# whwh747/A-Low-Texture-Robust-Hybrid-Feature-Based-Visual-Odometry

Measured on AMD Instinct MI355X. Metric: RGB-D frames/sec (640×480, 1k ORB + LSD + PEAC) at 1/2/4/8 GPUs, higher is better.
Workload: dtype u8/u16 integer + f32/f64; 1 GPU; 640x480 synthetic RGB-D, 1000 ORB (quota; 3/4 std + 1/4 lowtex scenes) + LSD lines + PEAC planes, 8192 frames per GPU per step (std640); frames_per_gpu=8192, parallelism=frames sharded, 1 rank(s), no data-path collective, distinct_frames=256, resident_bytes_per_frame_estimate=21100000

## Files before the change

a-low-texture-robust-hybrid-feature-based-visual-odometry_amd/__init__.py:

```python
import ctypes as C
import os
import subprocess
import numpy as np

_HERE = os.path.dirname(os.path.abspath(__file__))
_CSRC = os.path.join(_HERE, "csrc")
_LIBPATH = os.environ.get("HVO_LIB") or os.path.join(_CSRC, "libhvo.so")
_LIB = None
_LOADED_BEFORE_TORCH = False

HVO_OK = 0
STAGE_ORB, STAGE_LSD, STAGE_PLANES, STAGE_ALL = 1, 2, 4, 7
SLAB_LABELS = 1
STAGE_LSD_CULL = 8
STAGE_LINES3D, STAGE_VP, STAGE_PLANE_TAIL, STAGE_GRIDS = 16, 32, 64, 128
STAGE_FRAME = 1 | 2 | 8 | 4 | 16 | 32 | 64 | 128
LINE_MATCH_NNR, LINE_MATCH_BF, LINE_MATCH_DOUBLE = 0, 1, 2

KEYPOINT_DT = np.dtype([("x", "<f4"), ("y", "<f4"), ("size", "<f4"), ("angle", "<f4"),
                        ("response", "<f4"), ("octave", "<i4"), ("class_id", "<i4")])
KEYLINE_DT = np.dtype([("angle", "<f4"), ("class_id", "<i4"), ("octave", "<i4"),
                       ("pt_x", "<f4"), ("pt_y", "<f4"), ("response", "<f4"), ("size", "<f4"),
                       ("sx", "<f4"), ("sy", "<f4"), ("ex", "<f4"), ("ey", "<f4"),
                       ("sox", "<f4"), ("soy", "<f4"), ("eox", "<f4"), ("eoy", "<f4"),
# ... 1004 lines not shown

    def normals_lpvo(self, depth):
        depth = np.ascontiguousarray(depth, np.uint16); h, w = depth.shape
        cap = ((h + 14) // 15) * ((w + 14) // 15)
        nrm = np.zeros((cap, 3)); dz = np.zeros(cap, np.float32); px = np.zeros((cap, 2), np.int32); n = C.c_int(0)
        self._chk(lib().hvo_normals_lpvo(self.h, _p(depth), w, h, depth.strides[0], _p(nrm), _p(dz), _p(px), cap, C.byref(n)), "normals_lpvo")
        return nrm[: n.value], dz[: n.value], px[: n.value]

    def surface_normals(self, depth):
        depth = np.ascontiguousarray(depth, np.uint16); h, w = depth.shape
        cap = (((h + 2) // 3) // 2) * (((w + 2) // 3) // 2)
        out = np.zeros(max(cap, 1), SURFACE_NORMAL_DT); n = C.c_int(0)
        self._chk(lib().hvo_surface_normals(self.h, _p(depth), w, h, depth.strides[0], _p(out), cap, C.byref(n)), "surface_normals")
        return out[: n.value].copy()

    def peac_stats(self, frame=0):
        L = lib()
        L.hvo_debug_peac_stats.argtypes = [C.c_void_p, C.c_int, C.c_void_p]; L.hvo_debug_peac_stats.restype = C.c_int
        m = np.zeros(16, np.int32)
        self._chk(L.hvo_debug_peac_stats(self.h, frame, _p(m)), "peac_stats")
        return {"segments": int(m[0]), "coarse_planes": int(m[2]), "flags": int(m[3]), "planes": int(m[4]), "queue_entries": int(m[5]),
                "flood_rounds": int(m[8]), "flood_ranked_rounds": int(m[9]), "flood_serial_rounds": int(m[10]), "ahc_rounds": int(m[11]), "ahc_stops_no_head": int(m[12]), "ahc_stops_conflict": int(m[13]), "ahc_stops_key_order": int(m[14])}

    def hamming_matrix(self, q, t):
        q = np.ascontiguousarray(q, np.uint8).reshape(-1, 32); t = np.ascontiguousarray(t, np.uint8).reshape(-1, 32)
        d = np.zeros((len(q), len(t)), np.uint16)
        self._chk(lib().hvo_hamming_matrix(self.h, _p(q), len(q), _p(t), len(t), _p(d)), "hamming_matrix")
        return d

    def hamming_knn2(self, q, t):
# ... 835 lines not shown
```

a-low-texture-robust-hybrid-feature-based-visual-odometry_amd/csrc/lsd.hip:

```cpp
#include "hvo_internal.hpp"
#include <math.h>
#include <string.h>
#include <vector>
#include <algorithm>

#define LSD_PI 3.1415926535897932384626433832795
#define LSD_NOTDEF (-1024.0)
#ifndef LSD_RING
#define LSD_RING 256
#endif

static double lsd_sqrt_threshold(double rho)
{
    double c = rho * rho;
    while (sqrt(nextafter(c, INFINITY)) <= rho) c = nextafter(c, INFINITY);
    while (sqrt(c) > rho) c = nextafter(c, 0.0);
    return c;
}

struct LsdPlan {
    int w = 0, h = 0, sw = 0, sh = 0, batch = 0, nfeat = 0, nwords = 0;
    double *d_blur = nullptr;
    int chunk = 0;
    double4 *d_px = nullptr;
// ... 152 lines not shown
            const int rem = npend - 256;
            double ta = 0, tm = 0; int tp = 0;
            if (tid < rem) { ta = la[256 + tid]; tm = lm[256 + tid]; tp = lpos[256 + tid]; }
            __syncthreads();
            if (tid < rem) { la[tid] = ta; lm[tid] = tm; lpos[tid] = tp; }
            npend = rem;
            __syncthreads();
        }
        vprev = vcur; vprev_r = vcur_r;
    }
    if (tid < npend) emit(tid);
}

#define PRE_TW 192
#define PRE_SEG 96
__global__ __launch_bounds__(256) void k_lsd_pre(const uint8_t *__restrict__ gray, size_t gframe, int gpitch, int w, int h, int sw, int sh,
                                                 const int *__restrict__ xofs, const float *__restrict__ xa, const int *__restrict__ yofs, const float *__restrict__ yb,
                                                 double4 *__restrict__ px4, unsigned *__restrict__ defined, int nwords, double rhoT,
                                                 double k0, double k1, double k2, double k3, const int *__restrict__ redo_flags)
{
    if (redo_flags && !(redo_flags[blockIdx.z] & 4)) return;
    __shared__ double bl[4][256];
    __shared__ double sc[2][PRE_TW + 1];
    __shared__ double la[512], lm[512]; __shared__ int lpos[512];
    __shared__ int wcnt[4];
    const int tid = threadIdx.x, lane = tid & 63, wv = tid >> 6;
    const int x0 = blockIdx.x * PRE_TW, y0 = blockIdx.y * PRE_SEG, f = blockIdx.z;
    const uint8_t *G = gray + (size_t)f * gframe;
    double4 *PX = px4 + (size_t)f * sh * sw;
    const int xe = min(x0 + PRE_TW, sw - 1), ye = min(y0 + PRE_SEG, sh - 1);
    const int nsc = xe - x0 + 1;
    const int cA = xofs[x0], cB = min(xofs[xe] + 1, w - 1), ncols = cB - cA + 1;
    const int sya = yofs[y0] & 0xFFFF, syb = yofs[ye] >> 16;
    const bool colt = tid < ncols;
    const int x = min(cA + tid, w - 1);
    unsigned xm3 = (unsigned)refl(x - 3, w), xm2 = (unsigned)refl(x - 2, w), xm1 = (unsigned)refl(x - 1, w), x00 = (unsigned)x, xp1 = (unsigned)refl(x + 1, w), xp2 = (unsigned)refl(x + 2, w), xp3 = (unsigned)refl(x + 3, w);
    const int sxq = x0 + min(tid, nsc - 1);
    const int tx0 = xofs[sxq] - cA, tx1 = min(xofs[sxq] + 1, w - 1) - cA;
    const double a0 = (double)xa[2 * sxq], a1 = (double)xa[2 * sxq + 1];
    double v0 = 0, v1 = 0, v2 = 0, v3 = 0, v4 = 0, v5 = 0, v6 = 0;
    int ys = y0;
    int npend = 0;
    auto emit = [&](int i) {
        const float2 gq = reinterpret_cast<const float2 *>(la)[i];
        const double m = sqrt(lm[i]);
        const double aa = (double)fatan2_deg(gq.x, -gq.y) * (LSD_PI / 180);
        const double af = (double)(float)aa;
        double sn, cs; sincos(af, &sn, &cs);
        PX[lpos[i]] = make_double4(aa, cs, sn, m);
    };
    for (int j = sya - 3; j <= syb + 3; j++) {
        {
            const uint8_t *S = G + (size_t)refl(min(j, h + 2), h) * gpitch;
            asm("" : "+v"(xm3), "+v"(xm2), "+v"(xm1), "+v"(x00), "+v"(xp1), "+v"(xp2), "+v"(xp3));
            const unsigned q0 = S[xm3], q1 = S[xm2], q2 = S[xm1], q3 = S[x00], q4 = S[xp1], q5 = S[xp2], q6 = S[xp3];
            __builtin_amdgcn_sched_barrier(0);
            double s = k0 * (double)q0;
            s += k1 * (double)q1;
            s += k2 * (double)q2;
            s += k3 * (double)q3;
            s += k2 * (double)q4;
            s += k1 * (double)q5;
            s += k0 * (double)q6;
            v0 = v1; v1 = v2; v2 = v3; v3 = v4; v4 = v5; v5 = v6; v6 = s;
        }
        const int rb = j - 3;
        if (rb < sya) continue;
        {
            double s = k3 * v3;
            s += k2 * (v4 + v2);
            s += k1 * (v5 + v1);
            s += k0 * (v6 + v0);
            if (colt) bl[rb & 3][tid] = s;
        }
        __syncthreads();
        while (ys <= ye && (yofs[ys] >> 16) <= rb) {
            const int yo = yofs[ys];
            const int sy0 = yo & 0xFFFF, sy1 = yo >> 16;
            if (tid < nsc) {
                const double b0 = (double)yb[2 * ys], b1 = (double)yb[2 * ys + 1];
                const double *S0 = bl[sy0 & 3], *S1 = bl[sy1 & 3];
                const double t0 = S0[tx0] * a0 + S0[tx1] * a1;
                const double t1 = S1[tx0] * a0 + S1[tx1] * a1;
                sc[ys & 1][tid] = t0 * b0 + t1 * b1;
            }
            __syncthreads();
            if (ys > y0) {
                const int y = ys - 1, xg = x0 + tid;
                bool def = false;
                double xq = 0; float fgx = 0, fgy = 0;
                if (tid < PRE_TW && xg < sw - 1 && y < sh - 1) {
                    const double vprev = sc[y & 1][tid], vprev_r = sc[y & 1][tid + 1], vcur = sc[ys & 1][tid], vcur_r = sc[ys & 1][tid + 1];
                    const double DA = vcur_r - vprev, BC = vprev_r - vcur;
                    const double gx = DA + BC, gy = DA - BC;
                    xq = (gx * gx + gy * gy) / 4;
                    def = !(xq <= rhoT);
                    fgx = (float)gx; fgy = (float)gy;
                }
                const unsigned long long bal = __ballot(def);
                if (tid < PRE_TW && xg < ((sw + 31) & ~31)) {
                    const int word = (y * ((sw + 31) / 32)) + (xg >> 5);
                    if ((lane & 31) == 0) defined[(size_t)f * nwords + word] = (unsigned)(bal >> (lane & 32));
                }
                if (lane == 0) wcnt[wv] = __popcll(bal);
                __syncthreads();
                int base = 0, total = 0;
                for (int i = 0; i < 4; i++) { const int cn = wcnt[i]; if (i < wv) base += cn; total += cn; }
                if (def) { const int p = npend + base + __popcll(bal & ((1ull << lane) - 1)); reinterpret_cast<float2 *>(la)[p] = make_float2(fgx, fgy); lm[p] = xq; lpos[p] = y * sw + xg; }
                npend += total;
                if (npend >= 256) {
                    __syncthreads();
                    emit(tid);
                    const int rem = npend - 256;
                    double ta = 0, tm = 0; int tp = 0;
                    if (tid < rem) { ta = la[256 + tid]; tm = lm[256 + tid]; tp = lpos[256 + tid]; }
                    __syncthreads();
                    if (tid < rem) { la[tid] = ta; lm[tid] = tm; lpos[tid] = tp; }
                    npend = rem;
                }
            }
            __syncthreads();
            ys++;
        }
    }
    if (tid < npend) emit(tid);
}

__global__ __launch_bounds__(256) void k_lsd_prefix(const unsigned *__restrict__ defined, unsigned *__restrict__ defmask, unsigned *__restrict__ wprefix,
                                                    int *__restrict__ fcount, int nwords)
{
    __shared__ int wsum[4];
    const int f = blockIdx.x, tid = threadIdx.x, lane = tid & 63, wv = tid >> 6;
    const unsigned *D = defined + (size_t)f * nwords; unsigned *M = defmask + (size_t)f * nwords, *W = wprefix + (size_t)f * nwords;
    int run = 0;
    for (int base = 0; base < nwords; base += 256) {
        const int i = base + tid;
        const unsigned m = i < nwords ? D[i] : 0u;
        const int c = __popc(m);
        int incl = c;
#pragma unroll
// ... 631 lines not shown
    for (int j = 0; j < LBD_BLUR_ROWS + 2; j++) {
        const uint8_t *R = B + (size_t)refl(min(yb + j - 1, h), h) * w;
        const int a = R[xm], c = R[x], e = R[xp];
        hd[j] = e - a; hs[j] = a + 2 * c + e;
    }
#pragma unroll
    for (int j = 0; j < LBD_BLUR_ROWS; j++) {
        const int y = yb + j;
        if (y >= h) break;
        const int gx = hd[j] + 2 * hd[j + 1] + hd[j + 2];
        const int gy = hs[j + 2] - hs[j];
        dxy[((size_t)f * h + y) * w + x] = make_short2((short)gx, (short)gy);
    }
}

__global__ __launch_bounds__(256) void k_lbd_blur_sobel(const uint8_t *__restrict__ gray, size_t gframe, int gpitch,
                                                        short2 *__restrict__ dxy, int w, int h, int k0, int k1, int k2)
{
    const int nstrip = (w + 3) >> 2, item = blockIdx.x * 256 + threadIdx.x, f = blockIdx.z;
    const int rb = item / nstrip;
    const int x0 = (item - rb * nstrip) * 4, yb = rb * LBD_BLUR_ROWS;
    if (yb >= h) return;
    const uint8_t *G = gray + (size_t)f * gframe;
    const EdgeSel es = edge_sel(x0, w);
    const int o0 = max(x0 - 4, 0), o2 = min(x0 + 4, gpitch - 4);
    const unsigned kA = (unsigned)k0 | ((unsigned)k1 << 8) | ((unsigned)k2 << 16) | ((unsigned)k1 << 24);
    const int wv4 = w & ~3;
    const int v0 = max(yb - 1, 0), v1 = min(yb + LBD_BLUR_ROWS, h - 1);
    const int ylast = min(yb + LBD_BLUR_ROWS, h) - 1;
    int rs[5][6];
    int hd1[4], hs1[4], hd2[4], hs2[4];
#pragma unroll
    for (int j = 0; j < 4; j++) { hd1[j] = hs1[j] = hd2[j] = hs2[j] = 0; }
#pragma unroll
    for (int q = 0; q < 5; q++)
#pragma unroll
        for (int c = 0; c < 6; c++) rs[q][c] = 0;
    short2 *out = dxy + (size_t)f * h * w;
    const bool vecst = (w & 3) == 0;
    for (int sr = v0 - 2; sr <= v1 + 2; sr++) {
        const uint8_t *S = G + (size_t)refl(min(sr, h + 1), h) * gpitch;
        unsigned W0 = *reinterpret_cast<const uint32_t *>(S + o0), W1 = *reinterpret_cast<const uint32_t *>(S + x0),
                 W2 = *reinterpret_cast<const uint32_t *>(S + o2);
        edge_fix(es, W0, W1, W2);
#pragma unroll
        for (int q = 0; q < 4; q++)
#pragma unroll
            for (int c = 0; c < 6; c++) rs[q][c] = rs[q + 1][c];
        rs[4][0] = (int)__builtin_amdgcn_udot4(__builtin_amdgcn_alignbyte(W1, W0, 1), kA, (unsigned)k0 * ((W1 >> 8) & 0xFFu), false);
        rs[4][1] = (int)__builtin_amdgcn_udot4(__builtin_amdgcn_alignbyte(W1, W0, 2), kA, (unsigned)k0 * ((W1 >> 16) & 0xFFu), false);
        rs[4][2] = (int)__builtin_amdgcn_udot4(__builtin_amdgcn_alignbyte(W1, W0, 3), kA, (unsigned)k0 * (W1 >> 24), false);
        rs[4][3] = (int)__builtin_amdgcn_udot4(W1, kA, (unsigned)k0 * (W2 & 0xFFu), false);
        rs[4][4] = (int)__builtin_amdgcn_udot4(__builtin_amdgcn_alignbyte(W2, W1, 1), kA, (unsigned)k0 * ((W2 >> 8) & 0xFFu), false);
        rs[4][5] = (int)__builtin_amdgcn_udot4(__builtin_amdgcn_alignbyte(W2, W1, 2), kA, (unsigned)k0 * ((W2 >> 16) & 0xFFu), false);
        const int v = sr - 2;
        if (v < v0) continue;
        int bl[6];
#pragma unroll
        for (int c = 0; c < 6; c++) {
            const int sv = k0 * (rs[0][c] + rs[4][c]) + k1 * (rs[1][c] + rs[3][c]) + k2 * rs[2][c];
            int q;
            if (x0 - 1 + c < wv4) { q = sv >> 16; const int rem = sv & 0xFFFF; if (rem > 32768 || (rem == 32768 && (q & 1))) q++; }
            else q = (sv + 32768) >> 16;
            bl[c] = min(q, 255);
        }
        int hd0[4], hs0[4];
#pragma unroll
        for (int j = 0; j < 4; j++) {
            const int x = x0 + j;
            const int a = x == 0 ? bl[j + 2] : bl[j], e = x == w - 1 ? bl[j] : bl[j + 2];
            hd0[j] = e - a; hs0[j] = a + 2 * bl[j + 1] + e;
        }
        for (int pass = 0; pass < 2; pass++) {
            const int y = pass == 0 ? v - 1 : v;
            if (pass == 1 && !(v == h - 1)) break;
            if (y < yb || y > ylast) continue;
            short2 g[4];
#pragma unroll
            for (int j = 0; j < 4; j++) {
                int gx, gy;
                if (pass == 0) {
                    const int hdu = v >= 2 ? hd2[j] : hd0[j], hsu = v >= 2 ? hs2[j] : hs0[j];
                    gx = hdu + 2 * hd1[j] + hd0[j]; gy = hs0[j] - hsu;
                } else { gx = 2 * hd1[j] + 2 * hd0[j]; gy = 0; }
                g[j] = make_short2((short)gx, (short)gy);
            }
            short2 *o = out + (size_t)y * w + x0;
            if (vecst) *reinterpret_cast<uint4 *>(o) = *reinterpret_cast<const uint4 *>(g);
            else {
#pragma unroll
                for (int j = 0; j < 4; j++) if (x0 + j < w) o[j] = g[j];
            }
        }
#pragma unroll
        for (int j = 0; j < 4; j++) { hd2[j] = hd1[j]; hs2[j] = hs1[j]; hd1[j] = hd0[j]; hs1[j] = hs0[j]; }
    }
}

__constant__ int c_lbd_comb[32][2] = {
    { 0, 1 }, { 0, 2 }, { 0, 3 }, { 0, 4 }, { 0, 5 }, { 0, 6 }, { 1, 2 }, { 1, 3 }, { 1, 4 }, { 1, 5 }, { 1, 6 },
    { 2, 3 }, { 2, 4 }, { 2, 5 }, { 2, 6 }, { 2, 7 }, { 2, 8 }, { 3, 4 }, { 3, 5 }, { 3, 6 }, { 3, 7 }, { 3, 8 },
    { 4, 5 }, { 4, 6 }, { 4, 7 }, { 4, 8 }, { 5, 6 }, { 5, 7 }, { 5, 8 }, { 6, 7 }, { 6, 8 }, { 7, 8 } };

#define LBD_UNR 8
__global__ __launch_bounds__(64) void k_lbd_desc(const short2 *__restrict__ dxyImg, int w, int h,
                                                 const hvo_keyline *__restrict__ kls, const int *__restrict__ nkl, int kl_cap,
                                                 const float *__restrict__ gL, const float *__restrict__ gG, uint8_t *__restrict__ desc)
{
    __shared__ float rows[63][4];
    __shared__ float band[9][8];
    __shared__ float dv[72];
// ... 340 lines not shown
        sum = 1. / sum;
        for (int i = 0; i < 4; i++) P->k7[i] = k[i] * sum;
    }
    {
        float cf[5]; double sum = 0;
        for (int i = 0; i < 5; i++) { double x = i - 2.0; cf[i] = (float)exp(-0.5 * x * x); sum += cf[i]; }
        sum = 1. / sum;
        for (int i = 0; i < 3; i++) P->k5[i] = (int)lrintf((float)(cf[i] * sum) * 256.f);
    }
    {
        double u = (7 * 3 - 1) / 2, sigma = (7 * 2 + 1) / 2, inv = -1 / (2 * sigma * sigma);
        for (int i = 0; i < 21; i++) { double d = i - u; P->gL[i] = exp(d * d * inv); }
        u = (9 * 7 - 1) / 2; sigma = u; inv = -1 / (2 * sigma * sigma);
        for (int i = 0; i < 63; i++) { double d = i - u; P->gG[i] = exp(d * d * inv); }
    }
    std::vector<int> xofs(P->sw), yofs(P->sh); std::vector<float> xa(2 * P->sw), yb(2 * P->sh);
    const double scale = 1. / SCALE;
    for (int dx = 0; dx < P->sw; dx++) {
        float fx = (float)((dx + 0.5) * scale - 0.5); int sx = cvfloor_f(fx); fx -= sx;
        if (sx < 0) { fx = 0; sx = 0; }
        if (sx >= w - 1) { fx = 0; sx = w - 1; }
        xofs[dx] = sx; xa[2 * dx] = 1.f - fx; xa[2 * dx + 1] = fx;
    }
    for (int dy = 0; dy < P->sh; dy++) {
        float fy = (float)((dy + 0.5) * scale - 0.5); int sy = cvfloor_f(fy); fy -= sy;
        int sy0 = std::min(std::max(sy, 0), h - 1), sy1 = std::min(std::max(sy + 1, 0), h - 1);
        yofs[dy] = sy0 | (sy1 << 16); yb[2 * dy] = 1.f - fy; yb[2 * dy + 1] = fy;
    }
    std::vector<float> gLf(21), gGf(63);
    for (int i = 0; i < 21; i++) gLf[i] = (float)P->gL[i];
    for (int i = 0; i < 63; i++) gGf[i] = (float)P->gG[i];
// ... 17 lines not shown
    if (P->compact) {
        PA(P->d_px, CB * nsp * sizeof(double4));
        P->pool_cap = std::max<size_t>((size_t)((double)(B * nsp) * frac), 4096);
        PA(P->d_pool, P->pool_cap * sizeof(double4));
        PA(P->d_defmask, B * P->nwords * 4); PA(P->d_wprefix, B * P->nwords * 4);
        PA(P->d_fbase, B * 8); PA(P->d_fcount, B * 4); PA(P->d_pooltop, 16);
    } else
        PA(P->d_px, B * nsp * sizeof(double4));
    PA(P->d_defined, B * P->nwords * 4); PA(P->d_reg, B * nsp * 4);
    PA(P->d_segs, B * P->maxseg * 16); PA(P->d_kl_all, B * P->maxseg * sizeof(hvo_keyline));
    PA(P->d_kl, B * P->nfeat * sizeof(hvo_keyline)); PA(P->d_desc, B * P->nfeat * 32); PA(P->d_fn, B * P->nfeat * 24);
    PA(P->d_nkl, B * 4); PA(P->d_flags, B * 4);
    PA(P->d_kl2, B * P->nfeat * sizeof(hvo_keyline)); PA(P->d_desc2, B * P->nfeat * 32); PA(P->d_fn2, B * P->nfeat * 24); PA(P->d_nkl2, B * 4);
    if (P->kn.lbd_split.set) PA(P->d_b5, CB * npix);
    PA(P->d_dxy, CB * npix * sizeof(short2));
    PA(P->d_xofs, P->sw * 4); PA(P->d_yofs, P->sh * 4); PA(P->d_xa, P->sw * 8); PA(P->d_yb, P->sh * 8);
    PA(P->d_gL, 21 * 4); PA(P->d_gG, 63 * 4); PA(P->d_stats, B * 64);
    if (P->pre_fused) {
        int maxc = 0;
        for (int x0 = 0; x0 < P->sw; x0 += PRE_TW) { const int xe = std::min(x0 + PRE_TW, P->sw - 1); maxc = std::max(maxc, std::min(xofs[xe] + 1, w - 1) - xofs[x0] + 1); }
        if (maxc > 256) { P->pre_fused = false; PA(P->d_blur, CB * npix * 8); }
    }
#undef PA
    HVO_HIP(hipMemcpy(P->d_xofs, xofs.data(), P->sw * 4, hipMemcpyHostToDevice));
    HVO_HIP(hipMemcpy(P->d_yofs, yofs.data(), P->sh * 4, hipMemcpyHostToDevice));
    HVO_HIP(hipMemcpy(P->d_xa, xa.data(), P->sw * 8, hipMemcpyHostToDevice));
    HVO_HIP(hipMemcpy(P->d_yb, yb.data(), P->sh * 8, hipMemcpyHostToDevice));
    HVO_HIP(hipMemcpy(P->d_gL, gLf.data(), 21 * 4, hipMemcpyHostToDevice));
    HVO_HIP(hipMemcpy(P->d_gG, gGf.data(), 63 * 4, hipMemcpyHostToDevice));
    HVO_HIP(hipMemsetAsync(P->d_defined, 0, B * P->nwords * 4, ctx->s_lsd));
    HVO_HIP(hipMemsetAsync(P->d_nkl, 0, B * 4, ctx->s_lsd));
    HVO_HIP(hipMemsetAsync(P->d_nkl2, 0, B * 4, ctx->s_lsd));
    HVO_HIP(hipMemsetAsync(P->d_flags, 0, B * 4, ctx->s_lsd));
    HVO_HIP(hipDeviceSynchronize());
    return HVO_OK;
}

int lsd_prepare(hvo_ctx *ctx, int w, int h, int batch, bool culled, LsdView *v)
{
    int rc = lsd_ensure_plan(ctx, w, h, batch);
    if (rc) return rc;
    LsdPlan *P = plan_of(ctx);
// ... 136 lines not shown
    if (cull && P->nfeat > CULL_MAXL) return HVO_ERR_UNSUPPORTED;
    for (int c0 = 0; c0 < n; c0 += P->chunk) {
        const int m = std::min(P->chunk, n - c0);
        const uint8_t *gc = gray + (size_t)c0 * O.pyr_bytes;
        const size_t ko = (size_t)c0 * P->nfeat;
        id = hvo_prof_begin(ctx, "lbd_sobel", st);
        if (ctx->readings & HVO_READING_BLUR_FLOAT) {
            if (!P->d_b5) HVO_HIP(hipMalloc((void **)&P->d_b5, (size_t)P->chunk * w * h));
            if ((rc = readings_gblur_enqueue(st, gc, O.pyr_bytes, gpitch, w, h, P->d_b5, (size_t)w * h, w, m, 5, 1.0, true))) return rc;
            hipLaunchKernelGGL(k_lbd_sobel, dim3((w + 255) / 256, (h + LBD_BLUR_ROWS - 1) / LBD_BLUR_ROWS, m), dim3(256), 0, st, P->d_b5, P->d_dxy, w, h);
        } else
        if (P->d_b5) {
            hipLaunchKernelGGL(k_lbd_blur5, dim3((w + 255) / 256, (h + LBD_BLUR_ROWS - 1) / LBD_BLUR_ROWS, m), dim3(256), 0, st, gc, O.pyr_bytes, gpitch, P->d_b5, w, h, P->k5[0], P->k5[1], P->k5[2]);
            hipLaunchKernelGGL(k_lbd_sobel, dim3((w + 255) / 256, (h + LBD_BLUR_ROWS - 1) / LBD_BLUR_ROWS, m), dim3(256), 0, st, P->d_b5, P->d_dxy, w, h);
        } else
            hipLaunchKernelGGL(k_lbd_blur_sobel, dim3((((w + 3) / 4) * ((h + LBD_BLUR_ROWS - 1) / LBD_BLUR_ROWS) + 255) / 256, 1, m), dim3(256), 0, st, gc, O.pyr_bytes, gpitch, P->d_dxy, w, h,
                               P->k5[0], P->k5[1], P->k5[2]);
        hvo_prof_end(ctx, id);
        id = hvo_prof_begin(ctx, "lbd_desc", st);
        hipLaunchKernelGGL(k_lbd_desc, dim3(P->nfeat, m), dim3(64), 0, st, P->d_dxy, w, h, P->d_kl + ko, P->d_nkl + c0, P->nfeat, P->d_gL, P->d_gG, P->d_desc + ko * 32);
        hvo_prof_end(ctx, id);
        if (cull) {
            id = hvo_prof_begin(ctx, "lsd_cull", st);
            CullArgs c;
            c.kl = P->d_kl + ko; c.fn = P->d_fn + ko * 3; c.nkl = P->d_nkl + c0; c.tmp = P->d_kl_all + (size_t)c0 * P->maxseg; c.tmp_stride = P->maxseg;
            c.kl_out = P->d_kl2 + ko; c.fn_out = P->d_fn2 + ko * 3; c.nkl_out = P->d_nkl2 + c0;
            c.cap = P->nfeat; c.w = w; c.h = h; c.dis = ctx->cull_dis; c.cos_th = cos(ctx->cull_angle * 0.0174533); c.endpoint_dis = ctx->cull_endpoint;
            const int maxl = (P->nfeat + 63) & ~63;
            if (hvo_ensure_dyn_lds(reinterpret_cast<const void *>(k_cull_lines), cull_lds_bytes(maxl))) return HVO_ERR_HIP;
            hipLaunchKernelGGL(k_cull_lines, dim3(m), dim3(64), cull_lds_bytes(maxl), st, c, maxl);
            hipLaunchKernelGGL(k_lbd_desc, dim3(P->nfeat, m), dim3(64), 0, st, P->d_dxy, w, h, P->d_kl2 + ko, P->d_nkl2 + c0, P->nfeat, P->d_gL, P->d_gG, P->d_desc2 + ko * 32);
            hvo_prof_end(ctx, id);
// ... 104 lines not shown
        ok = hipDeviceSynchronize() == hipSuccess && hipMemcpy(list, d, (size_t)n * 4, hipMemcpyDeviceToHost) == hipSuccess &&
             hipMemcpy(n_kept, dn, 4, hipMemcpyDeviceToHost) == hipSuccess && hipMemcpy(released, dr, (size_t)width * height, hipMemcpyDeviceToHost) == hipSuccess;
    }
    (void)hipFree(d); (void)hipFree(dn); (void)hipFree(dr);
    return ok ? HVO_OK : HVO_ERR_HIP;
}

extern "C" int hvo_debug_lsd_stats(hvo_ctx *ctx, int frame, long long *out8)
{
    LsdPlan *P = ctx ? plan_of(ctx) : nullptr;
    if (!P || frame < 0 || frame >= P->batch) return HVO_ERR_INVALID_ARG;
    HVO_HIP(hipMemcpy(out8, P->d_stats + (size_t)frame * 8, 64, hipMemcpyDeviceToHost));
    return HVO_OK;
}

extern "C" int hvo_lsd_async_report(hvo_ctx *ctx, int *frames_regrown, int *foreign_workers, int *workers_per_frame)
{
    LsdPlan *P = ctx ? plan_of(ctx) : nullptr;
    if (!ctx) return HVO_ERR_INVALID_ARG;
    if (frames_regrown) *frames_regrown = 0;
    if (foreign_workers) *foreign_workers = 0;
    if (workers_per_frame) *workers_per_frame = 0;
    if (!P || !P->d_actl || P->async_last_n < 1) return HVO_OK;
    if (hipSetDevice(ctx->device) != hipSuccess) return HVO_ERR_NO_DEVICE;
    HVO_HIP(hipStreamSynchronize(hvo_stream_lsd(ctx)));
    int redo = 0;
    HVO_HIP(hipMemcpy(&redo, P->d_redo, 4, hipMemcpyDeviceToHost));
    std::vector<LaCtl> ctl((size_t)P->async_last_n);
    HVO_HIP(hipMemcpy(ctl.data(), P->d_actl, ctl.size() * sizeof(LaCtl), hipMemcpyDeviceToHost));
    int nf = 0;
// ... 15 lines not shown
```

Baseline: 55900 frames/s.

## Batch LSD preprocessing rows in chunks and widen fused LBD blur-sobel tile

```diff
diff --git a/a-low-texture-robust-hybrid-feature-based-visual-odometry_amd/__init__.py b/a-low-texture-robust-hybrid-feature-based-visual-odometry_amd/__init__.py
--- a/a-low-texture-robust-hybrid-feature-based-visual-odometry_amd/__init__.py
+++ b/a-low-texture-robust-hybrid-feature-based-visual-odometry_amd/__init__.py
@@ -1042,6 +1042,19 @@
         self._chk(lib().hvo_surface_normals(self.h, _p(depth), w, h, depth.strides[0], _p(out), cap, C.byref(n)), "surface_normals")
         return out[: n.value].copy()
 
+    def lsd_images(self, frame=0):
+        L = lib()
+        L.hvo_debug_lsd_images.argtypes = [C.c_void_p, C.c_int, C.POINTER(C.c_int), C.POINTER(C.c_int), C.c_void_p, C.c_void_p, C.c_longlong, C.POINTER(C.c_longlong), C.c_void_p]
+        L.hvo_debug_lsd_images.restype = C.c_int
+        w, h = self._w, self._h
+        sw, sh = int(round(w * 0.8)), int(round(h * 0.8))
+        mask = np.zeros((sh, (sw + 31) // 32), np.uint32); rec = np.zeros((sw * sh, 4), np.float64); dxy = np.zeros((h, w, 2), np.int16)
+        n = C.c_longlong(0); csw = C.c_int(0); csh = C.c_int(0)
+        self._chk(L.hvo_debug_lsd_images(self.h, frame, C.byref(csw), C.byref(csh), _p(mask), _p(rec), len(rec), C.byref(n), _p(dxy)), "lsd_images")
+        if (csw.value, csh.value) != (sw, sh):
+            raise HvoError(-1, "lsd_images: the plan's scaled size is %d x %d" % (csw.value, csh.value))
+        return {"mask": mask, "records": rec[:n.value].copy(), "dxy": dxy}
+
     def peac_stats(self, frame=0):
         L = lib()
         L.hvo_debug_peac_stats.argtypes = [C.c_void_p, C.c_int, C.c_void_p]; L.hvo_debug_peac_stats.restype = C.c_int
diff --git a/a-low-texture-robust-hybrid-feature-based-visual-odometry_amd/csrc/lsd.hip b/a-low-texture-robust-hybrid-feature-based-visual-odometry_amd/csrc/lsd.hip
--- a/a-low-texture-robust-hybrid-feature-based-visual-odometry_amd/csrc/lsd.hip
+++ b/a-low-texture-robust-hybrid-feature-based-visual-odometry_amd/csrc/lsd.hip
@@ -190,116 +190,144 @@
 
 #define PRE_TW 192
 #define PRE_SEG 96
+#define PRE_CH 4
+#define PRE_RING 8
+__attribute__((amdgpu_waves_per_eu(5)))
 __global__ __launch_bounds__(256) void k_lsd_pre(const uint8_t *__restrict__ gray, size_t gframe, int gpitch, int w, int h, int sw, int sh,
                                                  const int *__restrict__ xofs, const float *__restrict__ xa, const int *__restrict__ yofs, const float *__restrict__ yb,
                                                  double4 *__restrict__ px4, unsigned *__restrict__ defined, int nwords, double rhoT,
                                                  double k0, double k1, double k2, double k3, const int *__restrict__ redo_flags)
 {
     if (redo_flags && !(redo_flags[blockIdx.z] & 4)) return;
-    __shared__ double bl[4][256];
-    __shared__ double sc[2][PRE_TW + 1];
-    __shared__ double la[512], lm[512]; __shared__ int lpos[512];
-    __shared__ int wcnt[4];
-    const int tid = threadIdx.x, lane = tid & 63, wv = tid >> 6;
+    __shared__ double bl[PRE_RING][256];
+    __shared__ double sc[PRE_CH + 1][PRE_TW + 1];
+    __shared__ unsigned short qid[PRE_CH * PRE_TW];
+    __shared__ int qn[2];
+    const int tid = threadIdx.x, lane = tid & 63;
     const int x0 = blockIdx.x * PRE_TW, y0 = blockIdx.y * PRE_SEG, f = blockIdx.z;
     const uint8_t *G = gray + (size_t)f * gframe;
     double4 *PX = px4 + (size_t)f * sh * sw;
     const int xe = min(x0 + PRE_TW, sw - 1), ye = min(y0 + PRE_SEG, sh - 1);
     const int nsc = xe - x0 + 1;
-    const int cA = xofs[x0], cB = min(xofs[xe] + 1, w - 1), ncols = cB - cA + 1;
-    const int sya = yofs[y0] & 0xFFFF, syb = yofs[ye] >> 16;
-    const bool colt = tid < ncols;
+    const int cA = xofs[x0];
+    const int sya = yofs[y0] & 0xFFFF;
     const int x = min(cA + tid, w - 1);
     unsigned xm3 = (unsigned)refl(x - 3, w), xm2 = (unsigned)refl(x - 2, w), xm1 = (unsigned)refl(x - 1, w), x00 = (unsigned)x, xp1 = (unsigned)refl(x + 1, w), xp2 = (unsigned)refl(x + 2, w), xp3 = (unsigned)refl(x + 3, w);
-    const int sxq = x0 + min(tid, nsc - 1);
+    const int sci = min(tid, nsc - 1), sxq = x0 + sci;
     const int tx0 = xofs[sxq] - cA, tx1 = min(xofs[sxq] + 1, w - 1) - cA;
-    const double a0 = (double)xa[2 * sxq], a1 = (double)xa[2 * sxq + 1];
+    const float a0f = xa[2 * sxq], a1f = xa[2 * sxq + 1];
+    const int gi = min(tid, PRE_TW - 1);
+    const bool gcol = tid < PRE_TW && x0 + tid < sw - 1;
+    const bool wstore = (lane & 31) == 0 && tid < PRE_TW && x0 + tid < ((sw + 31) & ~31);
+    const bool whi = (lane & 32) != 0;
+    const int wpr = (sw + 31) / 32;
     double v0 = 0, v1 = 0, v2 = 0, v3 = 0, v4 = 0, v5 = 0, v6 = 0;
-    int ys = y0;
-    int npend = 0;
-    auto emit = [&](int i) {
-        const float2 gq = reinterpret_cast<const float2 *>(la)[i];
-        const double m = sqrt(lm[i]);
-        const double aa = (double)fatan2_deg(gq.x, -gq.y) * (LSD_PI / 180);
+    auto rowpass = [&](const uint8_t *S) {
+        asm("" : "+v"(xm3), "+v"(xm2), "+v"(xm1), "+v"(x00), "+v"(xp1), "+v"(xp2), "+v"(xp3));
+        const unsigned q0 = S[xm3], q1 = S[xm2], q2 = S[xm1], q3 = S[x00], q4 = S[xp1], q5 = S[xp2], q6 = S[xp3];
+        __builtin_amdgcn_sched_barrier(0);
+        double s = k0 * (double)q0;
+        s += k1 * (double)q1;
+        s += k2 * (double)q2;
+        s += k3 * (double)q3;
+        s += k2 * (double)q4;
+        s += k1 * (double)q5;
+        s += k0 * (double)q6;
+        v0 = v1; v1 = v2; v2 = v3; v3 = v4; v4 = v5; v5 = v6; v6 = s;
+    };
+    auto colpass = [&](int rb) {
+        double s = k3 * v3;
+        s += k2 * (v4 + v2);
+        s += k1 * (v5 + v1);
+        s += k0 * (v6 + v0);
+        bl[rb & (PRE_RING - 1)][tid] = s;
+    };
+    auto emit = [&](int i, int ybase) {
+        const int id = qid[i], s = id >> 8, t = id & 255;
+        const double vprev = sc[s][t], vprev_r = sc[s][t + 1], vcur = sc[s + 1][t], vcur_r = sc[s + 1][t + 1];
+        const double DA = vcur_r - vprev, BC = vprev_r - vcur;
+        const double gx = DA + BC, gy = DA - BC;
+        const double xq = (gx * gx + gy * gy) / 4;
+        const double m = sqrt(xq);
+        const double aa = (double)fatan2_deg((float)gx, -(float)gy) * (LSD_PI / 180);
         const double af = (double)(float)aa;
         double sn, cs; sincos(af, &sn, &cs);
-        PX[lpos[i]] = make_double4(aa, cs, sn, m);
+        PX[(size_t)(ybase + s) * sw + (x0 + t)] = make_double4(aa, cs, sn, m);
     };
-    for (int j = sya - 3; j <= syb + 3; j++) {
-        {
-            const uint8_t *S = G + (size_t)refl(min(j, h + 2), h) * gpitch;
-            asm("" : "+v"(xm3), "+v"(xm2), "+v"(xm1), "+v"(x00), "+v"(xp1), "+v"(xp2), "+v"(xp3));
-            const unsigned q0 = S[xm3], q1 = S[xm2], q2 = S[xm1], q3 = S[x00], q4 = S[xp1], q5 = S[xp2], q6 = S[xp3];
-            __builtin_amdgcn_sched_barrier(0);
-            double s = k0 * (double)q0;
-            s += k1 * (double)q1;
-            s += k2 * (double)q2;
-            s += k3 * (double)q3;
-            s += k2 * (double)q4;
-            s += k1 * (double)q5;
-            s += k0 * (double)q6;
-            v0 = v1; v1 = v2; v2 = v3; v3 = v4; v4 = v5; v5 = v6; v6 = s;
-        }
-        const int rb = j - 3;
-        if (rb < sya) continue;
-        {
-            double s = k3 * v3;
-            s += k2 * (v4 + v2);
-            s += k1 * (v5 + v1);
-            s += k0 * (v6 + v0);
-            if (colt) bl[rb & 3][tid] = s;
-        }
+    for (int j = sya - 3; j < sya + 3; j++) rowpass(G + (size_t)refl(min(j, h + 2), h) * gpitch);
+    int rbn = sya;
+    const uint8_t *Sp = G + (size_t)(sya + 3) * gpitch;
+    if (tid == 0) { qn[0] = 0; qn[1] = 0; }
+    double vlast = 0, tprev = 0;
+    int prow = -1, par = 0;
+    for (int ys = y0; ys <= ye; ys += PRE_CH) {
+        const int nr = min(PRE_CH, ye - ys + 1);
+        int yo[PRE_CH]; float wb[2 * PRE_CH];
+#pragma unroll
+        for (int r = 0; r < PRE_CH; r++) { yo[r] = yofs[ys + r]; wb[2 * r] = yb[2 * (ys + r)]; wb[2 * r + 1] = yb[2 * (ys + r) + 1]; }
+        const int rt = (nr == 4 ? yo[3] : nr == 3 ? yo[2] : nr == 2 ? yo[1] : yo[0]) >> 16;
+        const int rfast = min(rt, h - 4);
+        for (; rbn + 4 <= rfast; rbn += 5) {
+#pragma unroll
+            for (int u = 0; u < 5; u++) { rowpass(Sp); Sp += gpitch; colpass(rbn + u); }
+        }
+        for (; rbn <= rfast; rbn++) { rowpass(Sp); Sp += gpitch; colpass(rbn); }
+        for (; rbn <= rt; rbn++) { rowpass(G + (size_t)refl(min(rbn + 3, h + 2), h) * gpitch); colpass(rbn); }
         __syncthreads();
-        while (ys <= ye && (yofs[ys] >> 16) <= rb) {
-            const int yo = yofs[ys];
-            const int sy0 = yo & 0xFFFF, sy1 = yo >> 16;
-            if (tid < nsc) {
-                const double b0 = (double)yb[2 * ys], b1 = (double)yb[2 * ys + 1];
-                const double *S0 = bl[sy0 & 3], *S1 = bl[sy1 & 3];
-                const double t0 = S0[tx0] * a0 + S0[tx1] * a1;
+        if (tid == 0) qn[par ^ 1] = 0;
+        sc[0][sci] = vlast;
+        const double a0 = (double)a0f, a1 = (double)a1f;
+#pragma unroll
+        for (int r = 0; r < PRE_CH; r++) {
+            if (r < nr) {
+                const int sy0 = yo[r] & 0xFFFF, sy1 = yo[r] >> 16;
+                const double b0 = (double)wb[2 * r], b1 = (double)wb[2 * r + 1];
+                const double *S0 = bl[sy0 & (PRE_RING - 1)], *S1 = bl[sy1 & (PRE_RING - 1)];
+                double t0;
+                if (sy0 == prow) t0 = tprev; else t0 = S0[tx0] * a0 + S0[tx1] * a1;
                 const double t1 = S1[tx0] * a0 + S1[tx1] * a1;
-                sc[ys & 1][tid] = t0 * b0 + t1 * b1;
+                tprev = t1; prow = sy1;
+                vlast = t0 * b0 + t1 * b1;
+                sc[r + 1][sci] = vlast;
             }
-            __syncthreads();
-            if (ys > y0) {
-                const int y = ys - 1, xg = x0 + tid;
-                bool def = false;
-                double xq = 0; float fgx = 0, fgy = 0;
-                if (tid < PRE_TW && xg < sw - 1 && y < sh - 1) {
-                    const double vprev = sc[y & 1][tid], vprev_r = sc[y & 1][tid + 1], vcur = sc[ys & 1][tid], vcur_r = sc[ys & 1][tid + 1];
-                    const double DA = vcur_r - vprev, BC = vprev_r - vcur;
-                    const double gx = DA + BC, gy = DA - BC;
-                    xq = (gx * gx + gy * gy) / 4;
-                    def = !(xq <= rhoT);
-                    fgx = (float)gx; fgy = (float)gy;
+        }
+        __syncthreads();
+        const int s0 = ys == y0 ? 1 : 0, ybase = ys - 1;
+        double pl = sc[s0][gi], pr = sc[s0][gi + 1];
+        unsigned mw[PRE_CH];
+#pragma unroll
+        for (int s = 0; s < PRE_CH; s++) {
+            mw[s] = 0;
+            if (s >= s0 && s < nr) {
+                const double cl = sc[s + 1][gi], cr = sc[s + 1][gi + 1];
+                const double DA = cr - pl, BC = pr - cl;
+                const double gx = DA + BC, gy = DA - BC;
+                const double xq = (gx * gx + gy * gy) / 4;
+                const bool def = gcol && !(xq <= rhoT);
+                const unsigned long long bal = __ballot(def);
+                mw[s] = whi ? (unsigned)(bal >> 32) : (unsigned)bal;
+                if (bal) {
+                    int base = 0;
+                    if (lane == 0) base = atomicAdd(&qn[par], __popcll(bal));
+                    base = __builtin_amdgcn_readfirstlane(base);
+                    if (def) qid[base + __popcll(bal & ((1ull << lane) - 1))] = (unsigned short)((s << 8) | tid);
                 }
-                const unsigned long long bal = __ballot(def);
-                if (tid < PRE_TW && xg < ((sw + 31) & ~31)) {
-                    const int word = (y * ((sw + 31) / 32)) + (xg >> 5);
-                    if ((lane & 31) == 0) defined[(size_t)f * nwords + word] = (unsigned)(bal >> (lane & 32));
-                }
-                if (lane == 0) wcnt[wv] = __popcll(bal);
-                __syncthreads();
-                int base = 0, total = 0;
-                for (int i = 0; i < 4; i++) { const int cn = wcnt[i]; if (i < wv) base += cn; total += cn; }
-                if (def) { const int p = npend + base + __popcll(bal & ((1ull << lane) - 1)); reinterpret_cast<float2 *>(la)[p] = make_float2(fgx, fgy); lm[p] = xq; lpos[p] = y * sw + xg; }
-                npend += total;
-                if (npend >= 256) {
-                    __syncthreads();
-                    emit(tid);
-                    const int rem = npend - 256;
-                    double ta = 0, tm = 0; int tp = 0;
-                    if (tid < rem) { ta = la[256 + tid]; tm = lm[256 + tid]; tp = lpos[256 + tid]; }
-                    __syncthreads();
-                    if (tid < rem) { la[tid] = ta; lm[tid] = tm; lpos[tid] = tp; }
-                    npend = rem;
-                }
+                pl = cl; pr = cr;
             }
-            __syncthreads();
-            ys++;
-        }
-    }
-    if (tid < npend) emit(tid);
+        }
+        if (wstore) {
+            unsigned wcol = (unsigned)tid;
+            asm volatile("" : "+v"(wcol));
+            wcol = ((unsigned)x0 + wcol) >> 5;
+#pragma unroll
+            for (int s = 0; s < PRE_CH; s++)
+                if (s >= s0 && s < nr) (defined + (size_t)f * nwords + (size_t)(ybase + s) * wpr)[wcol] = mw[s];
+        }
+        __syncthreads();
+        const int n = qn[par];
+        for (int i = tid; i < n; i += 256) emit(i, ybase);
+        par ^= 1;
+    }
 }
 
 __global__ __launch_bounds__(256) void k_lsd_prefix(const unsigned *__restrict__ defined, unsigned *__restrict__ defmask, unsigned *__restrict__ wprefix,
@@ -961,87 +989,120 @@
     }
 }
 
+#define LBD_FUSED_ROWS 32
+template <bool AL>
+static __device__ __forceinline__ void lbd_blur_sobel_body(const uint8_t *__restrict__ G, int gpitch, short2 *__restrict__ out, int w, int h, int x0, int yb, int k0, int k1, int k2)
+{
+    const EdgeSel es = edge_sel(x0, w);
+    const unsigned o0 = (unsigned)max(x0 - 4, 0), o1 = (unsigned)x0, o2 = (unsigned)min(x0 + 4, gpitch - 4);
+    const unsigned kA = (unsigned)k0 | ((unsigned)k1 << 8) | ((unsigned)k2 << 16) | ((unsigned)k1 << 24);
+    const unsigned kB0 = (unsigned)k0, kB1 = (unsigned)k0 << 8, kB2 = (unsigned)k0 << 16, kB3 = (unsigned)k0 << 24;
+    const int v0 = max(yb - 1, 0), v1 = min(yb + LBD_FUSED_ROWS, h - 1);
+    const bool left = x0 == 0;
+    const int jr = w - 1 - x0;
+    const int hupT = !AL && x0 >= (w & ~3) ? 1 : 0, hup5 = !AL && x0 + 4 >= (w & ~3) ? 1 : 0;
+    int acc[4][6];
+    int k0b = k0, k1b = k1;
+    asm("" : "+s"(k0b), "+s"(k1b));
+#pragma unroll
+    for (int q = 0; q < 4; q++)
+#pragma unroll
+        for (int c = 0; c < 6; c++) acc[q][c] = 0;
+    int sr = v0 - 2;
+    auto step = [&](int (&s)[6]) {
+        const unsigned ro = __umul24((unsigned)refl(min(sr, h + 1), h), (unsigned)gpitch);
+        unsigned W0 = *reinterpret_cast<const uint32_t *>(G + (ro + o0)), W1 = *reinterpret_cast<const uint32_t *>(G + (ro + o1)),
+                 W2 = *reinterpret_cast<const uint32_t *>(G + (ro + o2));
+        edge_fix(es, W0, W1, W2);
+        sr++;
+        int r[6];
+        r[0] = (int)__builtin_amdgcn_udot4(__builtin_amdgcn_alignbyte(W1, W0, 1), kA, __builtin_amdgcn_udot4(W1, kB1, 0u, false), false);
+        r[1] = (int)__builtin_amdgcn_udot4(__builtin_amdgcn_alignbyte(W1, W0, 2), kA, __builtin_amdgcn_udot4(W1, kB2, 0u, false), false);
+        r[2] = (int)__builtin_amdgcn_udot4(__builtin_amdgcn_alignbyte(W1, W0, 3), kA, __builtin_amdgcn_udot4(W1, kB3, 0u, false), false);
+        r[3] = (int)__builtin_amdgcn_udot4(W1, kA, __builtin_amdgcn_udot4(W2, kB0, 0u, false), false);
+        r[4] = (int)__builtin_amdgcn_udot4(__builtin_amdgcn_alignbyte(W2, W1, 1), kA, __builtin_amdgcn_udot4(W2, kB1, 0u, false), false);
+        r[5] = (int)__builtin_amdgcn_udot4(__builtin_amdgcn_alignbyte(W2, W1, 2), kA, __builtin_amdgcn_udot4(W2, kB2, 0u, false), false);
+#pragma unroll
+        for (int c = 0; c < 6; c++) {
+            s[c] = acc[0][c] + (int)__umul24((unsigned)k0b, (unsigned)r[c]);
+            acc[0][c] = acc[1][c] + (int)__umul24((unsigned)k1b, (unsigned)r[c]);
+            acc[1][c] = acc[2][c] + (int)__umul24((unsigned)k2, (unsigned)r[c]);
+            acc[2][c] = acc[3][c] + (int)__umul24((unsigned)k1, (unsigned)r[c]);
+            acc[3][c] = (int)__umul24((unsigned)k0, (unsigned)r[c]);
+            asm("" : "+v"(s[c]), "+v"(acc[0][c]), "+v"(acc[1][c]), "+v"(acc[2][c]));
+        }
+    };
+    auto terms = [&](const int (&s)[6], unsigned (&n)[4]) {
+        int bl[6];
+#pragma unroll
+        for (int c = 0; c < 6; c++) bl[c] = min((s[c] + 32767 + (((s[c] >> 16) & 1) | (AL || c == 0 ? 0 : c == 5 ? hup5 : hupT))) >> 16, 255);
+        if (left) bl[0] = bl[2];
+        if (AL) { if (jr == 3) bl[5] = bl[3]; }
+        else {
+#pragma unroll
+            for (int j = 0; j < 4; j++) if (jr == j) bl[j + 2] = bl[j];
+        }
+#pragma unroll
+        for (int j = 0; j < 4; j++) n[j] = __builtin_amdgcn_perm((unsigned)(-(bl[j] + 2 * bl[j + 1] + bl[j + 2])), (unsigned)(bl[j + 2] - bl[j]), 0x05040100u);
+    };
+    typedef short lbd_s2 __attribute__((ext_vector_type(2)));
+    auto pk = [](unsigned u) { return __builtin_bit_cast(lbd_s2, u); };
+    auto store = [&](int y, const unsigned (&g)[4]) {
+        short2 *o = out + (size_t)y * w + x0;
+        if (AL) *reinterpret_cast<uint4 *>(o) = make_uint4(g[0], g[1], g[2], g[3]);
+        else {
+#pragma unroll
+            for (int j = 0; j < 4; j++) if (x0 + j < w) *reinterpret_cast<unsigned *>(o + j) = g[j];
+        }
+    };
+    const lbd_s2 two0 = { 2, 0 }, neg1 = { 1, -1 };
+    auto store_edge = [&](int y, const unsigned (&np)[4], const unsigned (&nq)[4]) {
+        unsigned g[4];
+#pragma unroll
+        for (int j = 0; j < 4; j++) g[j] = __builtin_bit_cast(unsigned, (lbd_s2)((pk(np[j]) + pk(nq[j])) * two0));
+        store(y, g);
+    };
+    auto rowstep = [&](int v, unsigned (&nP)[4], const unsigned (&nQ)[4]) {
+        int s[6]; unsigned n[4], g[4];
+        step(s);
+        terms(s, n);
+#pragma unroll
+        for (int j = 0; j < 4; j++) { g[j] = __builtin_bit_cast(unsigned, (lbd_s2)(pk(nQ[j]) * two0 + (pk(nP[j]) + pk(n[j]) * neg1))); nP[j] = n[j]; }
+        store(v - 1, g);
+    };
+    int s[6]; unsigned nA[4], nB[4];
+    if (h == 1) {
+        for (int i = 0; i < 5; i++) step(s);
+        terms(s, nA);
+#pragma unroll
+        for (int j = 0; j < 4; j++) nB[j] = 0;
+        store_edge(0, nA, nB);
+        return;
+    }
+    for (int i = 0; i < 5; i++) step(s);
+    terms(s, nA);
+    step(s);
+    terms(s, nB);
+    if (yb == 0) store_edge(0, nA, nB);
+    int v = v0 + 2;
+    for (; v < v1; v += 2) {
+        rowstep(v, nA, nB);
+        __builtin_amdgcn_sched_barrier(0);
+        rowstep(v + 1, nB, nA);
+    }
+    if (v == v1) rowstep(v, nA, nB);
+    if (yb + LBD_FUSED_ROWS >= h) store_edge(h - 1, nA, nB);
+}
+
+template <bool AL>
 __global__ __launch_bounds__(256) void k_lbd_blur_sobel(const uint8_t *__restrict__ gray, size_t gframe, int gpitch,
                                                         short2 *__restrict__ dxy, int w, int h, int k0, int k1, int k2)
 {
     const int nstrip = (w + 3) >> 2, item = blockIdx.x * 256 + threadIdx.x, f = blockIdx.z;
     const int rb = item / nstrip;
-    const int x0 = (item - rb * nstrip) * 4, yb = rb * LBD_BLUR_ROWS;
+    const int x0 = (item - rb * nstrip) * 4, yb = rb * LBD_FUSED_ROWS;
     if (yb >= h) return;
-    const uint8_t *G = gray + (size_t)f * gframe;
-    const EdgeSel es = edge_sel(x0, w);
-    const int o0 = max(x0 - 4, 0), o2 = min(x0 + 4, gpitch - 4);
-    const unsigned kA = (unsigned)k0 | ((unsigned)k1 << 8) | ((unsigned)k2 << 16) | ((unsigned)k1 << 24);
-    const int wv4 = w & ~3;
-    const int v0 = max(yb - 1, 0), v1 = min(yb + LBD_BLUR_ROWS, h - 1);
-    const int ylast = min(yb + LBD_BLUR_ROWS, h) - 1;
-    int rs[5][6];
-    int hd1[4], hs1[4], hd2[4], hs2[4];
-#pragma unroll
-    for (int j = 0; j < 4; j++) { hd1[j] = hs1[j] = hd2[j] = hs2[j] = 0; }
-#pragma unroll
-    for (int q = 0; q < 5; q++)
-#pragma unroll
-        for (int c = 0; c < 6; c++) rs[q][c] = 0;
-    short2 *out = dxy + (size_t)f * h * w;
-    const bool vecst = (w & 3) == 0;
-    for (int sr = v0 - 2; sr <= v1 + 2; sr++) {
-        const uint8_t *S = G + (size_t)refl(min(sr, h + 1), h) * gpitch;
-        unsigned W0 = *reinterpret_cast<const uint32_t *>(S + o0), W1 = *reinterpret_cast<const uint32_t *>(S + x0),
-                 W2 = *reinterpret_cast<const uint32_t *>(S + o2);
-        edge_fix(es, W0, W1, W2);
-#pragma unroll
-        for (int q = 0; q < 4; q++)
-#pragma unroll
-            for (int c = 0; c < 6; c++) rs[q][c] = rs[q + 1][c];
-        rs[4][0] = (int)__builtin_amdgcn_udot4(__builtin_amdgcn_alignbyte(W1, W0, 1), kA, (unsigned)k0 * ((W1 >> 8) & 0xFFu), false);
-        rs[4][1] = (int)__builtin_amdgcn_udot4(__builtin_amdgcn_alignbyte(W1, W0, 2), kA, (unsigned)k0 * ((W1 >> 16) & 0xFFu), false);
-        rs[4][2] = (int)__builtin_amdgcn_udot4(__builtin_amdgcn_alignbyte(W1, W0, 3), kA, (unsigned)k0 * (W1 >> 24), false);
-        rs[4][3] = (int)__builtin_amdgcn_udot4(W1, kA, (unsigned)k0 * (W2 & 0xFFu), false);
-        rs[4][4] = (int)__builtin_amdgcn_udot4(__builtin_amdgcn_alignbyte(W2, W1, 1), kA, (unsigned)k0 * ((W2 >> 8) & 0xFFu), false);
-        rs[4][5] = (int)__builtin_amdgcn_udot4(__builtin_amdgcn_alignbyte(W2, W1, 2), kA, (unsigned)k0 * ((W2 >> 16) & 0xFFu), false);
-        const int v = sr - 2;
-        if (v < v0) continue;
-        int bl[6];
-#pragma unroll
-        for (int c = 0; c < 6; c++) {
-            const int sv = k0 * (rs[0][c] + rs[4][c]) + k1 * (rs[1][c] + rs[3][c]) + k2 * rs[2][c];
-            int q;
-            if (x0 - 1 + c < wv4) { q = sv >> 16; const int rem = sv & 0xFFFF; if (rem > 32768 || (rem == 32768 && (q & 1))) q++; }
-            else q = (sv + 32768) >> 16;
-            bl[c] = min(q, 255);
-        }
-        int hd0[4], hs0[4];
-#pragma unroll
-        for (int j = 0; j < 4; j++) {
-            const int x = x0 + j;
-            const int a = x == 0 ? bl[j + 2] : bl[j], e = x == w - 1 ? bl[j] : bl[j + 2];
-            hd0[j] = e - a; hs0[j] = a + 2 * bl[j + 1] + e;
-        }
-        for (int pass = 0; pass < 2; pass++) {
-            const int y = pass == 0 ? v - 1 : v;
-            if (pass == 1 && !(v == h - 1)) break;
-            if (y < yb || y > ylast) continue;
-            short2 g[4];
-#pragma unroll
-            for (int j = 0; j < 4; j++) {
-                int gx, gy;
-                if (pass == 0) {
-                    const int hdu = v >= 2 ? hd2[j] : hd0[j], hsu = v >= 2 ? hs2[j] : hs0[j];
-                    gx = hdu + 2 * hd1[j] + hd0[j]; gy = hs0[j] - hsu;
-                } else { gx = 2 * hd1[j] + 2 * hd0[j]; gy = 0; }
-                g[j] = make_short2((short)gx, (short)gy);
-            }
-            short2 *o = out + (size_t)y * w + x0;
-            if (vecst) *reinterpret_cast<uint4 *>(o) = *reinterpret_cast<const uint4 *>(g);
-            else {
-#pragma unroll
-                for (int j = 0; j < 4; j++) if (x0 + j < w) o[j] = g[j];
-            }
-        }
-#pragma unroll
-        for (int j = 0; j < 4; j++) { hd2[j] = hd1[j]; hs2[j] = hs1[j]; hd1[j] = hd0[j]; hs1[j] = hs0[j]; }
-    }
+    lbd_blur_sobel_body<AL>(gray + (size_t)f * gframe, gpitch, dxy + (size_t)f * h * w, w, h, x0, yb, k0, k1, k2);
 }
 
 __constant__ int c_lbd_comb[32][2] = {
@@ -1412,7 +1473,7 @@
         u = (9 * 7 - 1) / 2; sigma = u; inv = -1 / (2 * sigma * sigma);
         for (int i = 0; i < 63; i++) { double d = i - u; P->gG[i] = exp(d * d * inv); }
     }
-    std::vector<int> xofs(P->sw), yofs(P->sh); std::vector<float> xa(2 * P->sw), yb(2 * P->sh);
+    std::vector<int> xofs(P->sw), yofs(P->sh + PRE_CH, 0); std::vector<float> xa(2 * P->sw), yb(2 * (P->sh + PRE_CH), 0.f);
     const double scale = 1. / SCALE;
     for (int dx = 0; dx < P->sw; dx++) {
         float fx = (float)((dx + 0.5) * scale - 0.5); int sx = cvfloor_f(fx); fx -= sx;
@@ -1460,18 +1521,20 @@
     PA(P->d_kl2, B * P->nfeat * sizeof(hvo_keyline)); PA(P->d_desc2, B * P->nfeat * 32); PA(P->d_fn2, B * P->nfeat * 24); PA(P->d_nkl2, B * 4);
     if (P->kn.lbd_split.set) PA(P->d_b5, CB * npix);
     PA(P->d_dxy, CB * npix * sizeof(short2));
-    PA(P->d_xofs, P->sw * 4); PA(P->d_yofs, P->sh * 4); PA(P->d_xa, P->sw * 8); PA(P->d_yb, P->sh * 8);
+    PA(P->d_xofs, P->sw * 4); PA(P->d_yofs, (P->sh + PRE_CH) * 4); PA(P->d_xa, P->sw * 8); PA(P->d_yb, (P->sh + PRE_CH) * 8);
     PA(P->d_gL, 21 * 4); PA(P->d_gG, 63 * 4); PA(P->d_stats, B * 64);
     if (P->pre_fused) {
         int maxc = 0;
         for (int x0 = 0; x0 < P->sw; x0 += PRE_TW) { const int xe = std::min(x0 + PRE_TW, P->sw - 1); maxc = std::max(maxc, std::min(xofs[xe] + 1, w - 1) - xofs[x0] + 1); }
-        if (maxc > 256) { P->pre_fused = false; PA(P->d_blur, CB * npix * 8); }
+        int maxr = 0;
+        for (int ys = 0; ys < P->sh; ys += PRE_CH) maxr = std::max(maxr, (yofs[std::min(ys + PRE_CH - 1, P->sh - 1)] >> 16) - (yofs[ys] & 0xFFFF) + 1);
+        if (maxc > 256 || maxr > PRE_RING) { P->pre_fused = false; PA(P->d_blur, CB * npix * 8); }
     }
 #undef PA
     HVO_HIP(hipMemcpy(P->d_xofs, xofs.data(), P->sw * 4, hipMemcpyHostToDevice));
-    HVO_HIP(hipMemcpy(P->d_yofs, yofs.data(), P->sh * 4, hipMemcpyHostToDevice));
+    HVO_HIP(hipMemcpy(P->d_yofs, yofs.data(), yofs.size() * 4, hipMemcpyHostToDevice));
     HVO_HIP(hipMemcpy(P->d_xa, xa.data(), P->sw * 8, hipMemcpyHostToDevice));
-    HVO_HIP(hipMemcpy(P->d_yb, yb.data(), P->sh * 8, hipMemcpyHostToDevice));
+    HVO_HIP(hipMemcpy(P->d_yb, yb.data(), yb.size() * 4, hipMemcpyHostToDevice));
     HVO_HIP(hipMemcpy(P->d_gL, gLf.data(), 21 * 4, hipMemcpyHostToDevice));
     HVO_HIP(hipMemcpy(P->d_gG, gGf.data(), 63 * 4, hipMemcpyHostToDevice));
     HVO_HIP(hipMemsetAsync(P->d_defined, 0, B * P->nwords * 4, ctx->s_lsd));
@@ -1638,8 +1701,11 @@
             hipLaunchKernelGGL(k_lbd_blur5, dim3((w + 255) / 256, (h + LBD_BLUR_ROWS - 1) / LBD_BLUR_ROWS, m), dim3(256), 0, st, gc, O.pyr_bytes, gpitch, P->d_b5, w, h, P->k5[0], P->k5[1], P->k5[2]);
             hipLaunchKernelGGL(k_lbd_sobel, dim3((w + 255) / 256, (h + LBD_BLUR_ROWS - 1) / LBD_BLUR_ROWS, m), dim3(256), 0, st, P->d_b5, P->d_dxy, w, h);
         } else
-            hipLaunchKernelGGL(k_lbd_blur_sobel, dim3((((w + 3) / 4) * ((h + LBD_BLUR_ROWS - 1) / LBD_BLUR_ROWS) + 255) / 256, 1, m), dim3(256), 0, st, gc, O.pyr_bytes, gpitch, P->d_dxy, w, h,
-                               P->k5[0], P->k5[1], P->k5[2]);
+{
+            const dim3 grid((((w + 3) / 4) * ((h + LBD_FUSED_ROWS - 1) / LBD_FUSED_ROWS) + 255) / 256, 1, m);
+            if ((w & 3) == 0) hipLaunchKernelGGL(k_lbd_blur_sobel<true>, grid, dim3(256), 0, st, gc, O.pyr_bytes, gpitch, P->d_dxy, w, h, P->k5[0], P->k5[1], P->k5[2]);
+            else hipLaunchKernelGGL(k_lbd_blur_sobel<false>, grid, dim3(256), 0, st, gc, O.pyr_bytes, gpitch, P->d_dxy, w, h, P->k5[0], P->k5[1], P->k5[2]);
+        }
         hvo_prof_end(ctx, id);
         id = hvo_prof_begin(ctx, "lbd_desc", st);
         hipLaunchKernelGGL(k_lbd_desc, dim3(P->nfeat, m), dim3(64), 0, st, P->d_dxy, w, h, P->d_kl + ko, P->d_nkl + c0, P->nfeat, P->d_gL, P->d_gG, P->d_desc + ko * 32);
@@ -1774,6 +1840,57 @@
     return HVO_OK;
 }
 
+extern "C" int hvo_debug_lsd_images(hvo_ctx *ctx, int frame, int *sw_out, int *sh_out, unsigned *mask, double *records, long long rec_cap, long long *n_records, short *dxy)
+{
+    LsdPlan *P = ctx ? plan_of(ctx) : nullptr;
+    if (!P || !mask || !records || !n_records || !dxy || rec_cap < 0) return HVO_ERR_INVALID_ARG;
+    if (!(ctx->last_stages & HVO_STAGE_LSD) || frame < 0 || frame >= ctx->batch_n) { ctx->last_error = "lsd images: no such frame in the last HVO_STAGE_LSD run"; return HVO_ERR_INVALID_ARG; }
+    if (ctx->batch_n > P->chunk || P->compact || (ctx->readings & (HVO_READING_LSD_8U | HVO_READING_BLUR_FLOAT))) {
+        ctx->last_error = "lsd images: only for a batch of at most one chunk with dense records and the default detector";
+        return HVO_ERR_UNSUPPORTED;
+    }
+    if (hipSetDevice(ctx->device) != hipSuccess) return HVO_ERR_NO_DEVICE;
+    OrbPlan &O = ctx->orb;
+    hipStream_t st = hvo_stream_lsd(ctx);
+    const int w = P->w, h = P->h, sw = P->sw, sh = P->sh, gpitch = O.lev[0].pitch;
+    const size_t nsp = (size_t)sw * sh;
+    const uint8_t *gray = O.d_pyr + O.lev[0].img_off + (size_t)frame * O.pyr_bytes;
+    double4 *px = P->d_px + (size_t)frame * nsp;
+    unsigned *def = P->d_defined + (size_t)frame * P->nwords;
+    HVO_HIP(hipStreamSynchronize(st));
+    std::vector<double> rec(nsp * 4);
+    HVO_HIP(hipMemcpy(rec.data(), px, nsp * sizeof(double4), hipMemcpyDeviceToHost));
+    HVO_HIP(hipMemcpy(dxy, P->d_dxy + (size_t)frame * w * h, (size_t)w * h * sizeof(short2), hipMemcpyDeviceToHost));
+    if (P->pre_fused)
+        hipLaunchKernelGGL(k_lsd_pre, dim3((sw + PRE_TW - 1) / PRE_TW, (sh - 1 + PRE_SEG - 1) / PRE_SEG, 1), dim3(256), 0, st, gray, O.pyr_bytes, gpitch,
+                           w, h, sw, sh, P->d_xofs, P->d_xa, P->d_yofs, P->d_yb, px, def, P->nwords, P->rhoT, P->k7[0], P->k7[1], P->k7[2], P->k7[3], (const int *)nullptr);
+    else {
+        hipLaunchKernelGGL(k_lsd_blur, dim3((w + 255) / 256, (h + LSD_BLUR_ROWS - 1) / LSD_BLUR_ROWS, 1), dim3(256), 0, st, gray, O.pyr_bytes, gpitch, P->d_blur, w, h,
+                           P->k7[0], P->k7[1], P->k7[2], P->k7[3]);
+        hipLaunchKernelGGL(k_lsd_resize_grad, dim3((((sw + 31) & ~31) + 255) / 256, (sh + GRAD_ROWS - 1) / GRAD_ROWS, 1), dim3(256), 0, st, P->d_blur, w, h, sw, sh,
+                           P->d_xofs, P->d_xa, P->d_yofs, P->d_yb, px, def, P->nwords, P->rho);
+    }
+    HVO_HIP(hipGetLastError());
+    HVO_HIP(hipStreamSynchronize(st));
+    HVO_HIP(hipMemcpy(mask, def, (size_t)P->nwords * 4, hipMemcpyDeviceToHost));
+    std::vector<double> rec2(nsp * 4);
+    HVO_HIP(hipMemcpy(rec2.data(), px, nsp * sizeof(double4), hipMemcpyDeviceToHost));
+    const int wpr = (sw + 31) / 32;
+    long long n = 0;
+    for (int y = 0; y < sh; y++)
+        for (int x = 0; x < sw; x++) {
+            if (!((mask[(size_t)y * wpr + (x >> 5)] >> (x & 31)) & 1u)) continue;
+            const size_t i = ((size_t)y * sw + x) * 4;
+            if (memcmp(&rec[i], &rec2[i], 32) != 0) { ctx->last_error = "lsd images: a record of the run differs from the one formed again"; return HVO_ERR_HIP; }
+            if (n < rec_cap) memcpy(records + n * 4, &rec[i], 32);
+            n++;
+        }
+    *n_records = n;
+    if (sw_out) *sw_out = sw;
+    if (sh_out) *sh_out = sh;
+    return HVO_OK;
+}
+
 extern "C" int hvo_lsd_async_report(hvo_ctx *ctx, int *frames_regrown, int *foreign_workers, int *workers_per_frame)
 {
     LsdPlan *P = ctx ? plan_of(ctx) : nullptr;
```

After: 58630 frames/s (median of 6 runs). 1.05x the previous value.
